# JoernZheng/parallel-data-compression-and-decompression

Hardware: AMD Instinct MI355X
Metric: compress+decompress GB/s (raw bytes / (deflate + inflate time)), .zwz bit-exact (higher is better)
Workload: dtype u8; 1 GPU; 10000 x 262144 B text-like files per GPU -> 50000 chunks of <=65535 B (BASELINE configs[2]); chunk_bytes=65535, max_batch_chunks=51200, parallelism=shard-per-gpu x1

## Files before the change

### parallel-data-compression-and-decompression_amd/csrc/lz_band.h

```cpp
#pragma once
#include "lz_core.h"

namespace zwz {

constexpr uint32_t kBand = kMaxChain;
constexpr uint32_t kBandNoLink = 0xffffu;
constexpr uint32_t kBandHaloWord = 0xffff0000u;

constexpr uint32_t kDenseSample = 2048;
ZWZ_HD bool sample_is_dense(uint32_t repeats, uint32_t thirds, uint32_t sampled, uint32_t L) {
    if (repeats == 0u || sampled == 0u) return false;
    if (thirds >= repeats) return true;
    const float walk = ((float)repeats + 3.0f * (float)thirds * (float)repeats / (float)(repeats - thirds)) * (float)L / ((float)sampled * (float)sampled);
    return walk >= 3.6f;
}

ZWZ_HD uint32_t band_word(uint32_t h, uint32_t p) { return h << 16 | p; }
ZWZ_HD uint32_t band_pos(uint32_t w) { return w & 0xffffu; }
ZWZ_HD uint32_t band_hash(uint32_t w) { return w >> 16; }

ZWZ_HD bool band_valid(uint32_t own, uint32_t c) {
    const uint32_t d = own - c;
    return (own ^ c) < 0x10000u && d < kMaxDist && d != band_pos(own);
}
ZWZ_HD bool band_first_at_max_dist(uint32_t own, uint32_t c) {
    const uint32_t p = band_pos(own), q = band_pos(c);
    return band_hash(c) == band_hash(own) && q != 0u && p - q == kMaxDist && !(p >= kSlidePos && q <= kWSize);
}

template <class Lv = LzDefaultLevel, class SFn>
ZWZ_HD uint32_t band_count(SFn S, uint32_t u) {
    const uint32_t own = S(u);
    uint32_t k = 0;
#if defined(__HIP_DEVICE_COMPILE__)
#pragma unroll
#endif
    for (uint32_t step = kBand; step >= 1u; step >>= 1) {
        const uint32_t t = k + step;
        if (t <= kBand && band_valid(own, S(u - t))) k = t;
    }
    if (k == 0u && band_first_at_max_dist(own, S(u - 1u))) k = 1u;
    return k < Lv::max_chain ? k : Lv::max_chain;
}

ZWZ_HD uint32_t band_ctz64(uint32_t lo, uint32_t hi) {
#if defined(__HIP_DEVICE_COMPILE__)
    uint32_t t0, t1;
    asm("v_ffbl_b32 %0, %1" : "=v"(t0) : "v"(lo));
    asm("v_ffbl_b32 %0, %1" : "=v"(t1) : "v"(hi));
    t1 |= 32u;
    return t0 < t1 ? t0 : t1;
#else
    if (lo) return (uint32_t)__builtin_ctz(lo);
    if (hi) return 32u + (uint32_t)__builtin_ctz(hi);
    return 0xffffffffu;
#endif
}
ZWZ_HD uint32_t band_key(uint32_t own_lo, uint32_t own_hi, uint32_t c_lo, uint32_t c_hi, uint32_t k) {
    const uint32_t t = band_ctz64(own_lo ^ c_lo, own_hi ^ c_hi);
    return ((t & 0x78u) << 5) | (129u - k);
}
ZWZ_HD uint32_t band_key_masked(uint32_t own_lo, uint32_t own_hi, uint32_t c_lo, uint32_t c_hi, uint32_t m_lo, uint32_t m_hi, uint32_t k) {
    const uint32_t t = band_ctz64((own_lo ^ c_lo) & m_lo, (own_hi ^ c_hi) & m_hi);
    return ((t & 0x78u) << 5) | (129u - k);
}
ZWZ_HD uint32_t band_tail_bytes(bool pure, uint32_t lookahead) {
    const uint32_t nb = pure ? lookahead - 3u : lookahead;
    return nb < 8u ? nb : 8u;
}
ZWZ_HD uint32_t band_tail_mask(uint32_t nbytes, uint32_t word ) {
    const uint32_t nb = nbytes > 4u * word ? nbytes - 4u * word : 0u;
    return nb >= 4u ? 0xffffffffu : (1u << (8u * nb)) - 1u;
}
constexpr uint32_t kBandKeyNonePure = 0u;
constexpr uint32_t kBandKeyNoneImpure = 0x2ffu;
ZWZ_HD uint32_t band_key_len(uint32_t key) { return key >> 8; }
ZWZ_HD uint32_t band_key_k(uint32_t key) { return 129u - (key & 0xffu); }

ZWZ_HD uint32_t band_record(uint32_t key, bool pure, uint32_t p, uint32_t cand_pos, uint32_t tail_len = 0) {
    const uint32_t len = band_key_len(key) == 15u ? tail_len : band_key_len(key) + (pure ? 3u : 0u), dist = p - cand_pos;
    if (len == kMinMatch && dist > kTooFar) return 0u;
    return entry_pack(len, dist);
}

template <class Lv = LzDefaultLevel, class SFn>
ZWZ_HD void band_generic(const uint8_t* data, SFn S, uint32_t u, uint32_t cnt, uint32_t L, uint32_t& e128, uint32_t& e32) {
    const uint32_t p = band_pos(S(u)), lookahead = L - p;
    const uint32_t max_len = lookahead < kMaxMatch ? lookahead : kMaxMatch, nice = lookahead < Lv::nice ? lookahead : Lv::nice;
    uint32_t best = kMinMatch - 1u, best_pos = 0, snap = 0xffffffffu;
    for (uint32_t k = 1; k <= cnt; k++) {
        const uint32_t c = band_pos(S(u - k));
        const uint32_t len = match_len_from(data, c, p, 0u, max_len);
        if (len > best) { best = len; best_pos = c; }
        if (k == Lv::snap_chain) snap = best >= kMinMatch ? entry_pack(best, p - best_pos) : 0u;
        if (best >= nice) break;
    }
    e128 = best >= kMinMatch ? entry_pack(best, p - best_pos) : 0u;
    e32 = snap != 0xffffffffu ? snap : e128;
    if (entry_len(e128) == kMinMatch && entry_dist(e128) > kTooFar) e128 = 0;
    if (entry_len(e32) == kMinMatch && entry_dist(e32) > kTooFar) e32 = 0;
}

template <class Lv = LzDefaultLevel, class SFn, class LinkFn, class EFn>
ZWZ_HD void band_deep(const uint8_t* data, SFn S, LinkFn link, EFn E, uint32_t first_own, uint32_t u, uint32_t cnt, uint32_t k1,
                      uint32_t deep, uint32_t L, uint64_t own , uint32_t& e128,
                      uint32_t& e32 ) {
    const uint32_t p = band_pos(S(u)), lookahead = L - p;
    const uint32_t max_len = lookahead < kMaxMatch ? lookahead : kMaxMatch, nice = lookahead < Lv::nice ? lookahead : Lv::nice;
    uint32_t best = 0, best_pos = 0, snap = 0xffffffffu;
    uint32_t j = u - k1;
    for (;;) {
        const uint32_t k = u - j;
        if (k > Lv::snap_chain && snap == 0xffffffffu) snap = best ? entry_pack(best, p - best_pos) : 0u;
        const uint32_t c = band_pos(S(j));
        const uint32_t len = match_len_from(data, c, p, deep, max_len);
        if (len > best) { best = len; best_pos = c; if (len >= nice) break; }
        if (j >= first_own) {
            const uint32_t j2 = link(j);
            if (j2 == kBandNoLink || u - j2 > cnt) break;
            j = j2;
        } else {
            uint32_t k2 = k + 1u;
            while (k2 <= cnt && E(u - k2) != own) k2++;
            if (k2 > cnt) break;
            j = u - k2;
        }
    }
    e128 = entry_pack(best, p - best_pos);
    if (k1 <= Lv::snap_chain) e32 = snap != 0xffffffffu ? snap : e128;
}

template <uint32_t H, class Lv = LzDefaultLevel, class SFn, class LinkFn, class EFn>
ZWZ_HD void band_deep_batched(const uint8_t* data, SFn S, LinkFn link, EFn E, uint32_t first_own, uint32_t u, uint32_t cnt, uint32_t k1,
                              uint32_t deep, uint32_t L, uint64_t own, uint32_t& e128, uint32_t& e32, uint32_t* visited = nullptr) {
    static_assert(H >= 1, "a batch holds a sharer");
    const uint32_t p = band_pos(S(u)), lookahead = L - p;
    const uint32_t max_len = lookahead < kMaxMatch ? lookahead : kMaxMatch, nice = lookahead < Lv::nice ? lookahead : Lv::nice;
    auto next = [&](uint32_t j) -> uint32_t {
        if (j >= first_own) {
            const uint32_t j2 = link(j);
            return j2 == kBandNoLink || u - j2 > cnt ? kBandNoLink : j2;
        }
        uint32_t k2 = u - j + 1u;
        while (k2 <= cnt && E(u - k2) != own) k2++;
        return k2 > cnt ? kBandNoLink : u - k2;
    };
    uint32_t best = 0, best_pos = 0, snap = 0xffffffffu, seen = 0;
    uint32_t j = u - k1;
    bool walking = true;
    while (walking) {
        uint32_t jv[H], len[H], nv = 1;
        jv[0] = j;
        for (uint32_t h = 1; h < H; h++) {
            const uint32_t j2 = next(jv[h - 1u]);
            if (j2 == kBandNoLink) break;
            jv[h] = j2; nv++;
        }
        for (uint32_t h = 0; h < nv; h++) len[h] = match_len_from(data, band_pos(S(jv[h])), p, deep, max_len);
        bool alive = true;
        for (uint32_t h = 0; h < nv; h++) {
            if (!alive) break;
            if (u - jv[h] > Lv::snap_chain && snap == 0xffffffffu) snap = best ? entry_pack(best, p - best_pos) : 0u;
            if (len[h] > best) { best = len[h]; best_pos = band_pos(S(jv[h])); }
            seen++;
            alive = best < nice;
        }
        j = alive && nv == H ? next(jv[H - 1u]) : kBandNoLink;
        walking = j != kBandNoLink;
    }
    if (visited) *visited = seen;
    e128 = entry_pack(best, p - best_pos);
    if (k1 <= Lv::snap_chain) e32 = snap != 0xffffffffu ? snap : e128;
}

}
```

### parallel-data-compression-and-decompression_amd/csrc/zwz_band.hip

```cpp
#include <hip/hip_runtime.h>

#include "lz_band.h"
#include "zwz_kernels.h"
#include "zwz_device.h"

#ifndef ZWZ_BAND_EXP
#define ZWZ_BAND_EXP 0
#endif

#if ZWZ_BAND_EXP & 16
#define ZWZ_STAMP(ph) do { if (tid == 0) { const uint64_t now_ = __builtin_amdgcn_s_memtime(); atomicAdd(&tickets[16 + (ph)], (uint32_t)((now_ - stamp_) >> 8)); stamp_ = now_; } } while (0)
#else
#define ZWZ_STAMP(ph) do { } while (0)
#endif

namespace zwz {

constexpr uint32_t kDenseThreads = 256;
__global__ __launch_bounds__(kDenseThreads) void lz_dense_list_kernel(const uint8_t* __restrict__ in, const uint64_t* __restrict__ in_off,
                                                                      const uint32_t* __restrict__ in_len, uint32_t n, uint32_t* __restrict__ link_stat,
                                                                      uint32_t force ) {
    __shared__ uint32_t s_set[kDenseThreads / 64][2048];
    const uint32_t wave = threadIdx.x >> 6, lane = lane_id();
    uint32_t* set = s_set[wave];
    for (uint32_t c = blockIdx.x * (kDenseThreads / 64u) + wave; c < n; c += gridDim.x * (kDenseThreads / 64u)) {
        const uint32_t L = in_len[c];
        bool dense = force == 2u && L != 0u;
        if (!dense && L >= kMinMatch) {
            for (uint32_t i = lane; i < 2048u; i += 64u) set[i] = 0;
            __builtin_amdgcn_fence(__ATOMIC_ACQ_REL, "wavefront");
            const uint32_t* d32 = reinterpret_cast<const uint32_t*>(in + in_off[c]);
            const uint32_t sampled = min(L - (kMinMatch - 1u), kDenseSample), nd = ((L + 15u) & ~15u) >> 2;
            uint32_t repeats = 0, thirds = 0;
            static_assert(kDenseSample == 2048, "eight trips of 256 positions, their loads asked for together");
            uint32_t w0[8], w1[8];
#pragma unroll
            for (uint32_t t = 0; t < 8; t++) {
                const uint32_t i = 64u * t + lane;
                w0[t] = 256u * t < sampled && i < nd ? d32[i] : 0u; w1[t] = 256u * t < sampled && i + 1u < nd ? d32[i + 1u] : 0u;
            }
#pragma unroll
            for (uint32_t t = 0; t < 8; t++) {
                if (256u * t >= sampled) break;
#pragma unroll
                for (uint32_t j = 0; j < 4; j++) {
                    const uint32_t x = j ? __builtin_amdgcn_alignbyte(w1[t], w0[t], j) : w0[t];
                    const uint32_t h = hash3(x & 0xffu, (x >> 8) & 0xffu, (x >> 16) & 0xffu);
                    const bool live = 256u * t + 4u * lane + j < sampled;
                    uint32_t old = 0, old2 = 0;
                    if (live) old = atomicOr(&set[h >> 5], 1u << (h & 31u));
                    const bool again = live && ((old >> (h & 31u)) & 1u);
                    if (again) old2 = atomicOr(&set[1024u + (h >> 5)], 1u << (h & 31u));
                    repeats += (uint32_t)__popcll(__builtin_amdgcn_ballot_w64(again));
                    thirds += (uint32_t)__popcll(__builtin_amdgcn_ballot_w64(again && ((old2 >> (h & 31u)) & 1u)));
                }
            }
            dense = sample_is_dense(repeats, thirds, sampled, L);
            __builtin_amdgcn_fence(__ATOMIC_ACQ_REL, "wavefront");
        }
        if (lane == 0) link_stat[c] = dense ? kDenseMark : 0u;
    }
}

__global__ __launch_bounds__(1024) void lz_lists_kernel(const uint32_t* __restrict__ in_len, const uint32_t* __restrict__ link_stat, uint32_t n,
                                                        uint32_t* __restrict__ dense_list, uint32_t* __restrict__ sparse_list, uint32_t* __restrict__ tickets) {
    __shared__ uint32_t s_d[16], s_s[16];
    const uint32_t tid = threadIdx.x, lane = lane_id(), wave = tid >> 6;
    uint32_t nd = 0, ns = 0;
    for (uint32_t c0 = 0; c0 < n; c0 += 1024u) {
        const uint32_t c = c0 + tid;
        const bool live = c < n && in_len[c] != 0u, dense = live && link_stat[c] == kDenseMark, sparse = live && !dense;
        const uint64_t md = __builtin_amdgcn_ballot_w64(dense), ms = __builtin_amdgcn_ballot_w64(sparse);
        if (lane == 0) { s_d[wave] = (uint32_t)__popcll(md); s_s[wave] = (uint32_t)__popcll(ms); }
        __syncthreads();
        uint32_t bd = nd, bs = ns, td = 0, ts = 0;
        for (uint32_t w = 0; w < 16u; w++) { bd += w < wave ? s_d[w] : 0u; bs += w < wave ? s_s[w] : 0u; td += s_d[w]; ts += s_s[w]; }
        if (dense) dense_list[bd + rank_in(md)] = c;
        if (sparse) sparse_list[bs + rank_in(ms)] = c;
        nd += td; ns += ts;
        __syncthreads();
    }
    if (tid == 0) { tickets[kTicketDenseCount] = nd; tickets[kTicketSparseCount] = ns; }
}

#ifndef ZWZ_SORT_DEPTH
#define ZWZ_SORT_DEPTH 16
#endif
constexpr uint32_t kSortDepth = ZWZ_SORT_DEPTH;
__global__ __launch_bounds__(kSortThreads) void lz_sort_kernel(const uint8_t* __restrict__ in, const uint64_t* __restrict__ in_off,
                                                               const uint32_t* __restrict__ in_len, const uint32_t* __restrict__ list,
                                                               uint32_t* __restrict__ tickets, uint32_t* __restrict__ sorted,
                                                               uint16_t* __restrict__ hbuf ,
                                                               uint32_t* __restrict__ scratch ) {
    __shared__ __attribute__((aligned(16))) uint32_t tab[16384];
    __shared__ uint32_t s_wsum[kSortThreads / 64];
    __shared__ uint32_t s_chunk;
    const uint32_t tid = threadIdx.x, lane = lane_id(), wave = __builtin_amdgcn_readfirstlane(tid >> 6);
    const uint32_t n_list = tickets[kTicketDenseCount];
    for (;;) {
        __syncthreads();
        if (tid == 0) s_chunk = atomicAdd(&tickets[kTicketSortNext], 1u);
        __syncthreads();
        const uint32_t t = s_chunk;
        if (t >= n_list) break;
        const uint32_t chunk = list[t];
        const uint32_t L = in_len[chunk];
        const uint32_t n = L >= kMinMatch ? L - (kMinMatch - 1u) : 0u;
        if (n == 0) continue;
        const uint32_t* d32 = reinterpret_cast<const uint32_t*>(in + in_off[chunk]);
        const uint32_t nd = ((L + 15u) & ~15u) >> 2;
        uint16_t* hb = hbuf + (size_t)chunk * kLinkStride;
        uint16_t* out = reinterpret_cast<uint16_t*>(sorted + (size_t)chunk * kSortedStride);
        {
            uint4* t4 = reinterpret_cast<uint4*>(tab);
            for (uint32_t i = tid; i < 4096u; i += kSortThreads) t4[i] = make_uint4(0, 0, 0, 0);
        }
        __syncthreads();
        {
            const uint4* d4 = reinterpret_cast<const uint4*>(d32);
            const uint32_t nv = nd >> 2;
#pragma unroll 1
            for (uint32_t i0 = tid; 16u * i0 < n; i0 += 8u * kSortThreads) {
                uint4 v[8]; uint32_t nx[8];
#pragma unroll
                for (uint32_t r = 0; r < 8; r++) {
                    const uint32_t i = i0 + r * kSortThreads;
                    v[r] = i < nv ? d4[i] : make_uint4(0, 0, 0, 0);
                    nx[r] = i + 1u < nv ? d32[4u * i + 4u] : 0u;
                }
#pragma unroll
                for (uint32_t r = 0; r < 8; r++) {
                    const uint32_t i = i0 + r * kSortThreads;
                    if (16u * i >= n) break;
                    const uint32_t w[5] = {v[r].x, v[r].y, v[r].z, v[r].w, nx[r]};
                    uint32_t h[16];
#pragma unroll
                    for (uint32_t j = 0; j < 16; j++) {
                        const uint32_t x = (j & 3u) ? __builtin_amdgcn_alignbyte(w[(j >> 2) + 1u], w[j >> 2], j & 3u) : w[j >> 2];
                        h[j] = hash3(x & 0xffu, (x >> 8) & 0xffu, (x >> 16) & 0xffu);
                        if (16u * i + j < n) atomicAdd(&tab[h[j] >> 1], (h[j] & 1u) ? 0x10000u : 1u);
                    }
#pragma unroll
                    for (uint32_t j = 0; j < 16; j++) h[j] = (h[j] >> 1) << 2 | (h[j] & 1u);
                    uint4* hb4 = reinterpret_cast<uint4*>(hb + 16u * i);
                    hb4[0] = make_uint4(h[0] | h[1] << 16, h[2] | h[3] << 16, h[4] | h[5] << 16, h[6] | h[7] << 16);
                    hb4[1] = make_uint4(h[8] | h[9] << 16, h[10] | h[11] << 16, h[12] | h[13] << 16, h[14] | h[15] << 16);
                }
            }
        }
        __syncthreads();
        {
            const uint32_t w_base = wave * 4096u;
            uint32_t tot = 0;
            for (uint32_t r = 0; r < 64u; r++) { const uint32_t v = tab[w_base + r * 64u + lane]; tot += (v & 0xffffu) + (v >> 16); }
            tot = wave_scan_incl(tot);
            if (lane == 63) s_wsum[wave] = tot;
            __syncthreads();
            uint32_t carry = 0;
            for (uint32_t i = 0; i < kSortThreads / 64u; i++) carry += i < wave ? s_wsum[i] : 0u;
            for (uint32_t r = 0; r < 64u; r++) {
                const uint32_t idx = w_base + r * 64u + lane;
                const uint32_t v = tab[idx], lo = v & 0xffffu, hi = v >> 16, own = lo + hi;
                const uint32_t incl = wave_scan_incl(own), ex = carry + incl - own;
                tab[idx] = ex | (ex + lo) << 16;
                carry += (uint32_t)__builtin_amdgcn_readlane((int)incl, 63);
            }
        }
        __syncthreads();
        if (wave == 0) {
            constexpr uint32_t K = kSortDepth;
            const uint32_t full = n / (64u * K);
            auto bump = [&](uint32_t w) { return atomicAdd(reinterpret_cast<uint32_t*>(reinterpret_cast<uint8_t*>(tab) + (w & 0xfffcu)), 1u << ((w & 1u) << 4)); };
            const uint16_t* hin = hb + lane;
            uint16_t* o = out + lane;
            uint32_t hv[K];
            auto ask = [&](uint32_t* h8) {
#pragma unroll
                for (uint32_t j = 0; j < K; j++) h8[j] = hin[j * 64u];
                hin += 64u * K;
            };
            if (full) ask(hv);
            uint32_t hp[K], op[K];
            for (uint32_t t = 0; t < full; t++) {
                uint32_t hn[K], old[K];
                if (t + 1u < full) ask(hn);
#pragma unroll
                for (uint32_t j = 0; j < K; j++) old[j] = bump(hv[j]);
                if (t) {
#pragma unroll
                    for (uint32_t j = 0; j < K; j++) o[j * 64u] = (uint16_t)(op[j] >> ((hp[j] & 1u) << 4));
                    o += 64u * K;
                }
#pragma unroll
                for (uint32_t j = 0; j < K; j++) { hp[j] = hv[j]; op[j] = old[j]; hv[j] = hn[j]; }
            }
            if (full) {
#pragma unroll
                for (uint32_t j = 0; j < K; j++) o[j * 64u] = (uint16_t)(op[j] >> ((hp[j] & 1u) << 4));
            }
            for (uint32_t p = full * 64u * K + lane; p - lane < n; p += 64u) {
                if (p < n) {
                    const uint32_t w = hb[p];
                    out[p] = (uint16_t)(bump(w) >> ((w & 1u) << 4));
                }
            }
        }
        if (scratch) {
            __syncthreads();
            uint4* o4 = reinterpret_cast<uint4*>(scratch + (size_t)chunk * kLazyScratchWords + kLazyBendOff);
            const uint4* t4 = reinterpret_cast<const uint4*>(tab);
            for (uint32_t i = tid; i < 4096u; i += kSortThreads) o4[i] = t4[i];
        }
    }
}

__global__ __launch_bounds__(kPlaceThreads) void lz_place_kernel(const uint32_t* __restrict__ in_len, const uint32_t* __restrict__ list,
                                                                 uint32_t* __restrict__ tickets, uint32_t* __restrict__ sorted) {
    extern __shared__ __attribute__((aligned(16))) uint8_t smem[];
    uint16_t* stage = reinterpret_cast<uint16_t*>(smem);
    __shared__ uint32_t s_chunk;
    const uint32_t tid = threadIdx.x;
    const uint32_t n_list = tickets[kTicketDenseCount];
    for (;;) {
        __syncthreads();
        if (tid == 0) s_chunk = atomicAdd(&tickets[kTicketPlaceNext], 1u);
        __syncthreads();
        const uint32_t t = s_chunk;
        if (t >= n_list) break;
        const uint32_t chunk = list[t];
        const uint32_t L = in_len[chunk];
        const uint32_t n = L >= kMinMatch ? L - (kMinMatch - 1u) : 0u;
        const uint4* d4 = reinterpret_cast<const uint4*>(sorted + (size_t)chunk * kSortedStride);
        uint4* o4 = reinterpret_cast<uint4*>(reinterpret_cast<uint16_t*>(sorted + (size_t)chunk * kSortedStride) + 65536);
        uint4 d[8];
#pragma unroll
        for (uint32_t r = 0; r < 8; r++) if (8u * (tid + kPlaceThreads * r) < n) d[r] = d4[tid + kPlaceThreads * r];
#pragma unroll
        for (uint32_t r = 0; r < 8; r++) {
            const uint32_t p0 = 8u * (tid + kPlaceThreads * r);
            const uint32_t dw[4] = {d[r].x, d[r].y, d[r].z, d[r].w};
#pragma unroll
            for (uint32_t j = 0; j < 8; j++) if (p0 + j < n) stage[(dw[j >> 1] >> (16u * (j & 1u))) & 0xffffu] = (uint16_t)(p0 + j);
        }
        __syncthreads();
        for (uint32_t i = tid; 8u * i < n; i += kPlaceThreads) o4[i] = reinterpret_cast<const uint4*>(stage)[i];
    }
}

constexpr uint32_t kBandArr = kBandTile + kBand;
constexpr uint32_t kBandDataBytes = 65536 + 64;
constexpr uint32_t kBandOffS = kBandDataBytes, kBandOffE = kBandOffS + kBandArr * 4, kBandOffCk = kBandOffE + kBandArr * 8,
                   kBandOffHas = kBandOffCk + kBandTile * 2;
static_assert(kBandOffHas + 8192 == kBandLdsBytes, "lz_match_band LDS layout");
static_assert(kBandTile % 64 == 0 && kBandOffE % 8 == 0 && kBandOffS % 16 == 0 && kBandOffCk % 16 == 0, "lz_match_band LDS alignment");
constexpr uint32_t kBandRuns = kBandTile / 8;

#ifndef ZWZ_BAND_WAVES
#define ZWZ_BAND_WAVES 4
#endif
#ifndef ZWZ_BAND_P2_BATCH
#define ZWZ_BAND_P2_BATCH 4
#endif
constexpr uint32_t kP2Batch = ZWZ_BAND_P2_BATCH;
static_assert(kP2Batch >= 1 && kP2Batch <= 32, "lz_match_band: sharers a batch");
template <class Lv>
__global__ __launch_bounds__(kBandThreads, ZWZ_BAND_WAVES) void lz_match_band_kernel(const uint8_t* __restrict__ in, const uint64_t* __restrict__ in_off,
                                                                    const uint32_t* __restrict__ in_len, const uint32_t* __restrict__ list,
                                                                    uint32_t* __restrict__ tickets, const uint32_t* __restrict__ sorted,
                                                                    uint2* __restrict__ entries, uint64_t* __restrict__ has128) {
    extern __shared__ __attribute__((aligned(16))) uint8_t smem[];
    uint8_t* sdata = smem;
    uint32_t* S = reinterpret_cast<uint32_t*>(smem + kBandOffS);
    uint2* E = reinterpret_cast<uint2*>(smem + kBandOffE);
    uint16_t* ck = reinterpret_cast<uint16_t*>(smem + kBandOffCk);
    uint32_t* hasb = reinterpret_cast<uint32_t*>(smem + kBandOffHas);
    uint16_t* flist = reinterpret_cast<uint16_t*>(E + kBand);
    __shared__ uint32_t s_chunk, s_grp[2], s_nflag, s_nrun;
    __shared__ uint16_t s_halo_link[kBand];
    __shared__ uint32_t s_bin[132];
    __shared__ uint16_t s_order[kBandRuns];
#if ZWZ_BAND_EXP & 16
    __shared__ uint64_t s_p2_start;
#endif
    const uint32_t tid = threadIdx.x, lane = lane_id(), wave = __builtin_amdgcn_readfirstlane(tid >> 6);
    const uint32_t n_list = tickets[kTicketDenseCount];
    for (uint32_t i = tid; i < 2048u; i += kBandThreads) hasb[i] = 0;
#if ZWZ_BAND_EXP & 16
    uint64_t stamp_ = __builtin_amdgcn_s_memtime();
#endif
    for (;;) {
        __syncthreads();
        ZWZ_STAMP(7);
        if (tid == 0) s_chunk = atomicAdd(&tickets[kTicketBandNext], 1u);
        __syncthreads();
        const uint32_t tk = s_chunk;
        if (tk >= n_list) break;
        const uint32_t chunk = list[tk];
        const uint32_t L = in_len[chunk];
        const uint32_t n = L >= kMinMatch ? L - (kMinMatch - 1u) : 0u;
        uint2* ent = entries + (size_t)chunk * kEntryStride;
        uint64_t* hm = has128 + (size_t)chunk * kMaskWords;
        const uint4* spos4 = reinterpret_cast<const uint4*>(reinterpret_cast<const uint16_t*>(sorted + (size_t)chunk * kSortedStride) + 65536);
        copy_vec16(reinterpret_cast<uint4*>(sdata), reinterpret_cast<const uint4*>(in + in_off[chunk]), (L + 15u) >> 4);
        ZWZ_STAMP(0);
        bool prev_pure = false;
        auto spos_of = [&](uint32_t a_) { return 8u * tid < kBandArr && 8u * tid + a_ >= kBand && 8u * tid + a_ - kBand < n ? spos4[(8u * tid + a_ - kBand) >> 3] : make_uint4(0, 0, 0, 0); };
        static_assert(kBandArr <= 8u * kBandThreads, "a thread holds eight of a tile's positions");
        uint4 v_next = spos_of(0u);
        for (uint32_t a = 0; a < n; a += kBandTile) {
            const uint32_t b = min(a + kBandTile, n), m = b - a + kBand;
            if (a < kBand) for (uint32_t i = tid; i < kBand - a; i += kBandThreads) S[i] = kBandHaloWord;
            if (tid == 0) { s_grp[0] = 0; s_grp[1] = 0; s_nflag = 0; s_nrun = 0; }
            if (tid < 132u) s_bin[tid] = 0;
            __syncthreads();
            bool mixed = false;
            {
                const uint32_t pw[4] = {v_next.x, v_next.y, v_next.z, v_next.w};
                if (8u * tid + a >= kBand) {
                    uint32_t prev_w = 0, prev_t = 0;
#pragma unroll
                    for (uint32_t j = 0; j < 8; j++) {
                        const uint32_t p = (pw[j >> 1] >> (16u * (j & 1u))) & 0xffffu;
                        const uint32_t* d = reinterpret_cast<const uint32_t*>(sdata) + (p >> 2);
                        const uint32_t w0 = d[0], w1 = d[1], w2 = d[2], w3 = d[3];
                        const uint32_t x = __builtin_amdgcn_alignbyte(w1, w0, p & 3u) & 0xffffffu;
                        const uint32_t word = band_word(hash3(x & 0xffu, (x >> 8) & 0xffu, x >> 16), p);
                        const bool up = (p & 3u) != 0u;
                        const uint32_t ea = up ? w1 : w0, eb = up ? w2 : w1, ec = up ? w3 : w2, sh = (p + 3u) & 3u;
                        if (8u * tid + j < m) {
                            S[8u * tid + j] = word;
                            E[8u * tid + j] = make_uint2(__builtin_amdgcn_alignbyte(eb, ea, sh), __builtin_amdgcn_alignbyte(ec, eb, sh));
                            if (j) mixed |= band_hash(word) == band_hash(prev_w) && x != prev_t;
                        }
                        prev_w = word; prev_t = x;
                    }
                }
                v_next = spos_of(a + kBandTile);
            }
            __syncthreads();
            ZWZ_STAMP(1);
            bool pure;
            {
                const uint32_t i = 8u * tid;
                if (i && i < m) {
                    const uint32_t w = S[i], wp = S[i - 1u];
                    const uint32_t tg = load_u32(sdata, band_pos(w)), tp = load_u32(sdata, band_pos(wp));
                    mixed |= w != kBandHaloWord && wp != kBandHaloWord && band_hash(w) == band_hash(wp) && ((tg ^ tp) & 0xffffffu) != 0u;
                }
                pure = !__syncthreads_or((int)mixed);
                if (!pure) {
                    for (uint32_t i2 = tid; i2 < m; i2 += kBandThreads) { const uint32_t q = band_pos(S[i2]); E[i2] = make_uint2(load_u32(sdata, q), load_u32(sdata, q + 4u)); }
                }
            }
            const uint32_t off = pure ? 3u : 0u, deep = pure ? 11u : 8u;
            auto Sf = [&](uint32_t i) { return S[i]; };
            ZWZ_STAMP(2);
            {
                constexpr uint32_t kOwnPer = (kBandTile + kBandThreads - 1) / kBandThreads;
                constexpr uint32_t kCap = Lv::max_chain;
                static_assert(kCap <= kBand && (kCap & (kCap - 1u)) == 0u, "the count is a binary search over [0, max_chain] inside the halo");
                uint32_t own[kOwnPer], k[kOwnPer];
#pragma unroll
                for (uint32_t j = 0; j < kOwnPer; j++) { const uint32_t i = kBand + tid + kBandThreads * j; own[j] = i < m ? S[i] : kBandHaloWord; k[j] = 0; }
                auto search_step = [&](uint32_t step) {
                    uint32_t c[kOwnPer];
#pragma unroll
                    for (uint32_t j = 0; j < kOwnPer; j++) { const uint32_t t = k[j] + step; c[j] = S[kBand + tid + kBandThreads * j - (t <= kCap ? t : 0u)]; }
#pragma unroll
                    for (uint32_t j = 0; j < kOwnPer; j++) { const uint32_t t = k[j] + step; if (t <= kCap && band_valid(own[j], c[j])) k[j] = t; }
                };
                search_step(kCap);
                bool open = false;
#pragma unroll
                for (uint32_t j = 0; j < kOwnPer; j++) open |= kBand + tid + kBandThreads * j < m && k[j] != kCap;
                if (__builtin_amdgcn_ballot_w64(open) != 0) {
#pragma unroll
                    for (uint32_t step = kCap / 2u; step >= 1u; step >>= 1) search_step(step);
                }
#pragma unroll
                for (uint32_t j = 0; j < kOwnPer; j++) {
                    const uint32_t i = kBand + tid + kBandThreads * j;
                    if (i < m) {
                        if (k[j] == 0u && band_first_at_max_dist(own[j], S[i - 1u])) k[j] = 1u;
                        ck[i - kBand] = (uint16_t)k[j];
                    }
                }
            }
            __syncthreads();
            ZWZ_STAMP(3);
            const bool halo_links = a == 0u || prev_pure == pure;
            if (tid < kBand) reinterpret_cast<uint16_t*>(S)[2u * tid + 1u] = a != 0u && halo_links ? s_halo_link[tid] : (uint16_t)kBandNoLink;
            prev_pure = pure;
            const uint32_t n_run = (b - a + 7u) >> 3;
            uint32_t run_key = 0;
            if (tid < n_run) {
                const uint4 c8 = *reinterpret_cast<const uint4*>(ck + 8u * tid);
                const uint32_t cw[4] = {c8.x, c8.y, c8.z, c8.w};
#pragma unroll
                for (uint32_t j = 0; j < 8; j++) if (8u * tid + j < b - a) run_key = max(run_key, (cw[j >> 1] >> (16u * (j & 1u))) & 0xffu);
                if (run_key) atomicAdd(&s_bin[128u - run_key], 1u);
            }
            __syncthreads();
            if (wave == 0) {
                const uint32_t v0 = s_bin[lane], v1 = s_bin[64u + lane];
                const uint32_t i0 = wave_scan_incl(v0), t0 = (uint32_t)__builtin_amdgcn_readlane((int)i0, 63);
                const uint32_t i1 = wave_scan_incl(v1);
                s_bin[lane] = i0 - v0; s_bin[64u + lane] = t0 + i1 - v1;
                if (lane == 63) s_nrun = t0 + i1;
            }
            __syncthreads();
            if (tid < n_run && run_key) s_order[atomicAdd(&s_bin[128u - run_key], 1u)] = (uint16_t)tid;
            __syncthreads();
            ZWZ_STAMP(8);
            const uint32_t n_act = s_nrun, n_grp = (n_act + 7u) >> 3;
            const uint32_t none = pure ? kBandKeyNonePure : kBandKeyNoneImpure;
            for (;;) {
                uint32_t g = 0;
                if (lane == 0) g = atomicAdd(&s_grp[0], 1u);
                g = __builtin_amdgcn_readfirstlane(g);
                if (g >= n_grp) break;
                const uint32_t ri = 8u * g + (lane >> 3);
                const uint32_t i = kBand + 8u * (ri < n_act ? (uint32_t)s_order[ri] : 0u) + (lane & 7u);
                const bool active = ri < n_act && i < m;
                const uint32_t w = S[i], p = band_pos(w);
                const uint32_t cntb = active ? (uint32_t)ck[i - kBand] : 0u;
                const uint2 own = E[i];
                const uint32_t kmax = (ZWZ_BAND_EXP & 2) ? 0u : (uint32_t)__builtin_amdgcn_readlane((int)wave_scan_max_incl(cntb), 63);
                const uint32_t kmin = 128u - (uint32_t)__builtin_amdgcn_readlane((int)wave_scan_max_incl(cntb ? 128u - cntb : 0u), 63);
                uint32_t best = cntb ? none : 0xffffffffu, snap = none;
                const uint2* Ei = E + i;
                auto key_of = [&](const uint2 c, uint32_t kc) {
                    uint32_t t0, t1, a1, key;
                    asm("v_ffbl_b32 %0, %1" : "=v"(t0) : "v"(own.x ^ c.x));
                    asm("v_ffbl_b32 %0, %1" : "=v"(t1) : "v"(own.y ^ c.y));
                    asm("v_and_or_b32 %0, %1, %2, 32" : "=v"(a1) : "v"(t1), "s"(0x78u));
                    const uint32_t m8 = min(t0 & 0x78u, a1);
                    asm("v_lshl_or_b32 %0, %1, 5, %2" : "=v"(key) : "v"(m8), "s"(kc));
                    return key;
                };
                const uint32_t la = L - p;
                const bool tail = active && la < deep;
                if (__builtin_amdgcn_ballot_w64(tail) == 0) {
                    uint32_t k0 = 0;
                    for (; k0 + 8u <= kmin; k0 += 8u) {
                        uint2 c[8];
#pragma unroll
                        for (uint32_t j = 0; j < 8; j++) c[j] = Ei[-(int)(k0 + j + 1u)];
#pragma unroll
                        for (uint32_t j = 0; j < 8; j += 2) {
                            const uint32_t ka = key_of(c[j], 128u - k0 - j), kb = key_of(c[j + 1], 127u - k0 - j);
                            asm("v_max3_u32 %0, %0, %1, %2" : "+v"(best) : "v"(ka), "v"(kb));
                        }
                        if (k0 + 8u == Lv::snap_chain) snap = best;
                    }
                    for (; k0 < kmax; k0 += 8u) {
                        uint2 c[8];
#pragma unroll
                        for (uint32_t j = 0; j < 8; j++) c[j] = Ei[-(int)(k0 + j + 1u)];
#pragma unroll
                        for (uint32_t j = 0; j < 8; j++) {
                            const uint32_t key = key_of(c[j], 128u - k0 - j);
                            best = max(best, k0 + j + 1u <= cntb ? key : 0u);
                        }
                        if (k0 + 8u == Lv::snap_chain) snap = best;
                    }
                } else {
                    const uint32_t nb = tail ? band_tail_bytes(pure, la) : 8u, m_lo = band_tail_mask(nb, 0), m_hi = band_tail_mask(nb, 1);
                    for (uint32_t k = 1; k <= kmax; k++) {
                        const uint2 c = Ei[-(int)k];
                        const uint32_t key = band_key_masked(own.x, own.y, c.x, c.y, m_lo, m_hi, k);
                        best = max(best, k <= cntb ? key : 0u);
                        if (k == Lv::snap_chain) snap = best;
                    }
                }
                if (cntb == 0u) best = none;
                const uint32_t key32 = cntb > Lv::snap_chain ? snap : best;
                uint32_t e128 = 0, e32 = 0, k1 = 0;
                if (best != none) {
                    if (band_key_len(best) == 15u && !tail && !(ZWZ_BAND_EXP & 1)) k1 = band_key_k(best);
                    else e128 = band_record(best, pure, p, band_pos(S[i - band_key_k(best)]), la);
                }
                if (key32 != none && (tail || band_key_len(key32) != 15u)) e32 = band_record(key32, pure, p, band_pos(S[i - band_key_k(key32)]), la);
                if (active) {
                    if (k1) {
                        ck[i - kBand] = (uint16_t)(cntb | k1 << 8);
                        reinterpret_cast<uint16_t*>(S)[2u * i + 1u] = (uint16_t)(i - k1);
                        if (k1 > Lv::snap_chain && !(ZWZ_BAND_EXP & 4)) reinterpret_cast<uint32_t*>(ent + p)[1] = e32;
                        atomicOr(&hasb[p >> 5], 1u << (p & 31u));
                    } else {
                        reinterpret_cast<uint16_t*>(S)[2u * i + 1u] = (uint16_t)kBandNoLink;
                        if (e128) {
                            if (!(ZWZ_BAND_EXP & 4)) ent[p] = make_uint2(e128, e32); else asm volatile("" :: "v"(e128), "v"(e32), "v"(p));
                            atomicOr(&hasb[p >> 5], 1u << (p & 31u));
                        }
                    }
                }
            }
            for (uint32_t i = kBand + tid; i < m; i += kBandThreads) if ((uint32_t)ck[i - kBand] == 0u) reinterpret_cast<uint16_t*>(S)[2u * i + 1u] = (uint16_t)kBandNoLink;
            __syncthreads();
            ZWZ_STAMP(4);
            for (uint32_t i = kBand + tid; i - tid < m; i += kBandThreads) {
                const bool f = i < m && ((uint32_t)ck[i - kBand] >> 8) != 0u;
                const uint64_t fm = __builtin_amdgcn_ballot_w64(f);
                if (fm) {
                    uint32_t base = 0;
                    if (lane == 0) base = atomicAdd(&s_nflag, (uint32_t)__popcll(fm));
                    base = __builtin_amdgcn_readfirstlane(base);
                    if (f) flist[base + rank_in(fm)] = (uint16_t)i;
                }
            }
#if ZWZ_BAND_EXP & 16
            if (tid == 0) s_p2_start = __builtin_amdgcn_s_memtime();
#endif
            __syncthreads();
            ZWZ_STAMP(9);
            const uint32_t n_flag = s_nflag;
            for (;;) {
                uint32_t g = 0;
                if (lane == 0) g = atomicAdd(&s_grp[1], 1u);
                g = __builtin_amdgcn_readfirstlane(g);
                if (64u * g >= n_flag) break;
#if ZWZ_BAND_EXP & 16
                if (lane == 0 && g == ((n_flag + 63u) >> 6) / 2u) atomicAdd(&tickets[16 + 10], (uint32_t)((__builtin_amdgcn_s_memtime() - s_p2_start) >> 8));
#endif
                const bool on = 64u * g + lane < n_flag;
                const uint32_t i = on ? (uint32_t)flist[64u * g + lane] : kBand;
                const uint32_t c = ck[i - kBand], cnt = c & 0xffu, k1 = c >> 8;
                const uint32_t p = band_pos(S[i]), la = L - p;
                const uint32_t max_len = la < kMaxMatch ? la : kMaxMatch, nice = la < Lv::nice ? la : Lv::nice;
                const uint32_t own2_lo = load_u32(sdata, p + deep), own2_hi = load_u32(sdata, p + deep + 4u);
                const uint32_t own3_lo = load_u32(sdata, p + deep + 8u), own3_hi = load_u32(sdata, p + deep + 12u);
                uint32_t best = 0, best_pos = 0, snap = 0xffffffffu;
                uint32_t j = on ? i - k1 : kBand;
                uint32_t w = S[j];
                bool walking = on, slow = false;
                while (__builtin_amdgcn_ballot_w64(walking) != 0) {
                    uint32_t wv[kP2Batch], nv = walking ? 1u : 0u;
                    wv[0] = w;
                    bool more = walking;
#pragma unroll
                    for (uint32_t h = 1; h < kP2Batch; h++) {
                        const uint32_t link = wv[h - 1u] >> 16;
                        more = more && i - link <= cnt;
                        wv[h] = S[more ? link : kBand];
                        nv += more ? 1u : 0u;
                    }
                    const uint32_t link_n = wv[kP2Batch - 1u] >> 16;
                    const bool more_n = more && i - link_n <= cnt;
                    const uint32_t wn = S[more_n ? link_n : kBand];
                    bool alive = walking;
                    uint32_t jh = j;
#pragma unroll
                    for (uint32_t h = 0; h < kP2Batch; h++) {
                        const uint32_t q = band_pos(wv[h]), sh = (q + deep) & 3u;
                        const uint32_t* d = reinterpret_cast<const uint32_t*>(sdata) + ((q + deep) >> 2);
                        const uint32_t d0 = d[0], d1 = d[1], d2 = d[2], d3 = d[3], d4 = d[4];
                        uint32_t t0, t1, t2, t3;
                        asm("v_ffbl_b32 %0, %1" : "=v"(t0) : "v"(__builtin_amdgcn_alignbyte(d1, d0, sh) ^ own2_lo));
                        asm("v_ffbl_b32 %0, %1" : "=v"(t1) : "v"(__builtin_amdgcn_alignbyte(d2, d1, sh) ^ own2_hi));
                        asm("v_ffbl_b32 %0, %1" : "=v"(t2) : "v"(__builtin_amdgcn_alignbyte(d3, d2, sh) ^ own3_lo));
                        asm("v_ffbl_b32 %0, %1" : "=v"(t3) : "v"(__builtin_amdgcn_alignbyte(d4, d3, sh) ^ own3_hi));
                        const uint32_t tm = min(min(t0, t1 | 32u), min(t2 | 64u, t3 | 96u));
                        bool v = alive && h < nv;
                        if (!halo_links) { slow = slow || (v && jh < kBand); v = v && jh >= kBand; }
                        uint32_t l = deep + (tm >> 3);
                        if (v && tm == 0xffffffffu) l = match_len_from(sdata, q, p, deep + 16u, max_len);
                        l = l < max_len ? l : max_len;
                        if (v && i - jh > Lv::snap_chain && snap == 0xffffffffu) snap = best ? entry_pack(best, p - best_pos) : 0u;
                        if (v && l > best) { best = l; best_pos = q; }
                        alive = v && best < nice;
                        jh = wv[h] >> 16;
                    }
                    walking = alive && more_n;
                    j = link_n; w = wn;
                }
                uint32_t e128 = entry_pack(best, p - best_pos), e32 = snap != 0xffffffffu ? snap : e128;
                if (slow) {
                    const uint64_t own = (uint64_t)load_u32(sdata, p + off) | (uint64_t)load_u32(sdata, p + off + 4u) << 32;
                    band_deep<Lv>(sdata, Sf, [&](uint32_t jj) { return S[jj] >> 16; },
                              [&](uint32_t jj) { const uint2 e = E[jj]; return (uint64_t)e.x | (uint64_t)e.y << 32; },
                              kBand, i, cnt, k1, deep, L, own, e128, e32);
                }
                if (on) {
                    if (ZWZ_BAND_EXP & 4) asm volatile("" :: "v"(e128), "v"(e32), "v"(p));
                    if (!(ZWZ_BAND_EXP & 4)) {
                        reinterpret_cast<uint32_t*>(ent + p)[0] = e128;
                        if (k1 <= Lv::snap_chain) reinterpret_cast<uint32_t*>(ent + p)[1] = e32;
                    }
                }
            }
            __syncthreads();
            if (tid < kBand && b < n) {
                const uint32_t lk = S[m - kBand + tid] >> 16;
                s_halo_link[tid] = (uint16_t)(lk != kBandNoLink && lk >= m - kBand ? lk - (m - kBand) : kBandNoLink);
            }
            __syncthreads();
            ZWZ_STAMP(5);
        }
        __syncthreads();
        for (uint32_t i = tid; i < ((L + 63u) >> 6); i += kBandThreads) {
            hm[i] = (uint64_t)hasb[2 * i] | ((uint64_t)hasb[2 * i + 1] << 32);
            hasb[2 * i] = 0; hasb[2 * i + 1] = 0;
        }
        ZWZ_STAMP(6);
    }
}

uint32_t exp_flags_band() { return (uint32_t)(ZWZ_BAND_EXP); }

hipError_t configure_band_kernels() {
    hipError_t e = hipFuncSetAttribute(reinterpret_cast<const void*>(lz_place_kernel), hipFuncAttributeMaxDynamicSharedMemorySize, (int)kPlaceLdsBytes);
    if (e != hipSuccess) return e;
    e = hipFuncSetAttribute(reinterpret_cast<const void*>(lz_match_band_kernel<LzLevel<4>>), hipFuncAttributeMaxDynamicSharedMemorySize, (int)kBandLdsBytes);
    if (e != hipSuccess) return e;
    e = hipFuncSetAttribute(reinterpret_cast<const void*>(lz_match_band_kernel<LzLevel<5>>), hipFuncAttributeMaxDynamicSharedMemorySize, (int)kBandLdsBytes);
    if (e != hipSuccess) return e;
    return hipFuncSetAttribute(reinterpret_cast<const void*>(lz_match_band_kernel<LzLevel<6>>), hipFuncAttributeMaxDynamicSharedMemorySize, (int)kBandLdsBytes);
}

hipError_t launch_dense_list(const DeflateArgs& a, hipStream_t s, uint32_t which) {
    const uint32_t cus = a.cu_count ? a.cu_count : 256u, want = (a.n + kDenseThreads / 64u - 1u) / (kDenseThreads / 64u);
    hipLaunchKernelGGL(lz_dense_list_kernel, dim3(want < 8u * cus ? want : 8u * cus), dim3(kDenseThreads), 0, s, a.in, a.in_off, a.in_len, a.n, a.link_stat, which);
    hipLaunchKernelGGL(lz_lists_kernel, dim3(1), dim3(1024), 0, s, a.in_len, a.link_stat, a.n, a.dense_list, a.sparse_list, a.tickets);
    return hipGetLastError();
}

hipError_t launch_sort(const DeflateArgs& a, hipStream_t s) {
    const uint32_t cus = a.cu_count ? a.cu_count : 256u;
    const uint32_t G = a.n < 2u * cus ? a.n : 2u * cus;
    hipLaunchKernelGGL(lz_sort_kernel, dim3(G), dim3(kSortThreads), 0, s, a.in, a.in_off, a.in_len, a.dense_list, a.tickets, a.sorted, a.links,
                       reinterpret_cast<uint32_t*>(a.entries));
    return hipGetLastError();
}

hipError_t launch_place(const DeflateArgs& a, hipStream_t s) {
    const uint32_t cus = a.cu_count ? a.cu_count : 256u;
    const uint32_t G = a.n < cus ? a.n : cus;
    hipLaunchKernelGGL(lz_place_kernel, dim3(G), dim3(kPlaceThreads), kPlaceLdsBytes, s, a.in_len, a.dense_list, a.tickets, a.sorted);
    return hipGetLastError();
}

hipError_t launch_match_band(const DeflateArgs& a, hipStream_t s) {
    const uint32_t cus = a.cu_count ? a.cu_count : 256u;
    const uint32_t G = a.n < cus ? a.n : cus;
    switch (a.level) {
#define ZWZ_BAND_LAUNCH(N) case N: hipLaunchKernelGGL(lz_match_band_kernel<LzLevel<N>>, dim3(G), dim3(kBandThreads), kBandLdsBytes, s, a.in, a.in_off, a.in_len, a.dense_list, \
                                                 a.tickets, a.sorted, a.entries, a.has128); break;
        ZWZ_BAND_LAUNCH(4) ZWZ_BAND_LAUNCH(5) ZWZ_BAND_LAUNCH(6)
#undef ZWZ_BAND_LAUNCH
        default: return hipErrorInvalidValue;
    }
    return hipGetLastError();
}

}
```

Measured before the change: 22.22 GB/s.

## Pack two band-key candidates per VGPR with 16-bit SDWA ops and parameterise run size

New measurement: 23.36 GB/s, median of 6. 5.1% higher.

```diff
diff --git a/parallel-data-compression-and-decompression_amd/csrc/lz_band.h b/parallel-data-compression-and-decompression_amd/csrc/lz_band.h
--- a/parallel-data-compression-and-decompression_amd/csrc/lz_band.h
+++ b/parallel-data-compression-and-decompression_amd/csrc/lz_band.h
@@ -64,6 +64,40 @@
     const uint32_t t = band_ctz64((own_lo ^ c_lo) & m_lo, (own_hi ^ c_hi) & m_hi);
     return ((t & 0x78u) << 5) | (129u - k);
 }
+constexpr uint32_t kBandPairLenMask = 0x00780078u;
+ZWZ_HD uint32_t band_key_pair(uint32_t own_lo, uint32_t own_hi, uint32_t a_lo, uint32_t a_hi, uint32_t b_lo, uint32_t b_hi, uint32_t k, uint32_t mask) {
+    const uint32_t ta = band_ctz64(own_lo ^ a_lo, own_hi ^ a_hi) & 0xffffu, tb = band_ctz64(own_lo ^ b_lo, own_hi ^ b_hi) & 0xffffu;
+    return (((ta | tb << 16) & mask) << 5) | (129u - k) | (128u - k) << 16;
+}
+ZWZ_HD uint64_t band_trip_mask(uint32_t k0, uint32_t cnt) {
+    const int32_t over = (int32_t)(k0 + 8u) - (int32_t)cnt;
+    const uint32_t d = over < 0 ? 0u : over > 8 ? 8u : (uint32_t)over;
+    return 0x7878787878787878ull >> (8u * d < 63u ? 8u * d : 63u);
+}
+ZWZ_HD uint32_t band_pair_mask(uint64_t trip_mask, uint32_t j) {
+    return ((uint32_t)(trip_mask >> (8u * j)) & 0xffu) | ((uint32_t)(trip_mask >> (8u * j + 8u)) & 0xffu) << 16;
+}
+ZWZ_HD uint32_t band_pair_max(uint32_t pair) { return (pair & 0xffffu) > (pair >> 16) ? pair & 0xffffu : pair >> 16; }
+template <class Lv = LzDefaultLevel, class EFn>
+ZWZ_HD void band_first_pass(uint64_t own, EFn E, uint32_t cnt, uint32_t kmin, uint32_t kmax, uint32_t none, uint32_t& best, uint32_t& snap) {
+    const uint32_t own_lo = (uint32_t)own, own_hi = (uint32_t)(own >> 32);
+    uint32_t best2 = cnt ? none | none << 16 : 0xffffffffu;
+    snap = none;
+    for (uint32_t k0 = 0; k0 < kmax; k0 += 8u) {
+        const bool masked = k0 + 8u > kmin;
+        const uint64_t have = band_trip_mask(k0, cnt);
+        for (uint32_t j = 0; j < 8u; j += 2u) {
+            const uint64_t a = E(k0 + j + 1u), b = E(k0 + j + 2u);
+            const uint32_t key = band_key_pair(own_lo, own_hi, (uint32_t)a, (uint32_t)(a >> 32), (uint32_t)b, (uint32_t)(b >> 32), k0 + j + 1u,
+                                               masked ? band_pair_mask(have, j) : kBandPairLenMask);
+            const uint32_t lo = (key & 0xffffu) > (best2 & 0xffffu) ? key & 0xffffu : best2 & 0xffffu, hi = (key >> 16) > (best2 >> 16) ? key >> 16 : best2 >> 16;
+            best2 = lo | hi << 16;
+        }
+        if (k0 + 8u == Lv::snap_chain) snap = band_pair_max(best2);
+    }
+    best = cnt ? band_pair_max(best2) : none;
+}
+
 ZWZ_HD uint32_t band_tail_bytes(bool pure, uint32_t lookahead) {
     const uint32_t nb = pure ? lookahead - 3u : lookahead;
     return nb < 8u ? nb : 8u;
diff --git a/parallel-data-compression-and-decompression_amd/csrc/zwz_band.hip b/parallel-data-compression-and-decompression_amd/csrc/zwz_band.hip
--- a/parallel-data-compression-and-decompression_amd/csrc/zwz_band.hip
+++ b/parallel-data-compression-and-decompression_amd/csrc/zwz_band.hip
@@ -253,7 +253,13 @@
                    kBandOffHas = kBandOffCk + kBandTile * 2;
 static_assert(kBandOffHas + 8192 == kBandLdsBytes, "lz_match_band LDS layout");
 static_assert(kBandTile % 64 == 0 && kBandOffE % 8 == 0 && kBandOffS % 16 == 0 && kBandOffCk % 16 == 0, "lz_match_band LDS alignment");
-constexpr uint32_t kBandRuns = kBandTile / 8;
+#ifndef ZWZ_BAND_RUN
+#define ZWZ_BAND_RUN 8
+#endif
+constexpr uint32_t kBandRun = ZWZ_BAND_RUN;
+static_assert(kBandRun == 8 || kBandRun == 4 || kBandRun == 2, "lz_match_band: a run is 8, 4 or 2 entries");
+constexpr uint32_t kBandRuns = kBandTile / kBandRun, kBandRunsPer = (kBandRuns + kBandThreads - 1) / kBandThreads;
+static_assert(kBandLdsBytes + 1072u + 2u * kBandRuns <= 160u * 1024u, "lz_match_band: s_order does not fit beside the tile");
 
 #ifndef ZWZ_BAND_WAVES
 #define ZWZ_BAND_WAVES 4
@@ -391,14 +397,21 @@
             const bool halo_links = a == 0u || prev_pure == pure;
             if (tid < kBand) reinterpret_cast<uint16_t*>(S)[2u * tid + 1u] = a != 0u && halo_links ? s_halo_link[tid] : (uint16_t)kBandNoLink;
             prev_pure = pure;
-            const uint32_t n_run = (b - a + 7u) >> 3;
-            uint32_t run_key = 0;
-            if (tid < n_run) {
-                const uint4 c8 = *reinterpret_cast<const uint4*>(ck + 8u * tid);
-                const uint32_t cw[4] = {c8.x, c8.y, c8.z, c8.w};
-#pragma unroll
-                for (uint32_t j = 0; j < 8; j++) if (8u * tid + j < b - a) run_key = max(run_key, (cw[j >> 1] >> (16u * (j & 1u))) & 0xffu);
-                if (run_key) atomicAdd(&s_bin[128u - run_key], 1u);
+            const uint32_t n_run = (b - a + kBandRun - 1u) / kBandRun;
+            uint32_t run_key[kBandRunsPer];
+#pragma unroll
+            for (uint32_t t = 0; t < kBandRunsPer; t++) {
+                const uint32_t r = tid + kBandThreads * t;
+                run_key[t] = 0;
+                if (r < n_run) {
+                    uint32_t cw[4] = {0, 0, 0, 0};
+                    if constexpr (kBandRun == 8) { const uint4 c8 = *reinterpret_cast<const uint4*>(ck + 8u * r); cw[0] = c8.x; cw[1] = c8.y; cw[2] = c8.z; cw[3] = c8.w; }
+                    else if constexpr (kBandRun == 4) { const uint2 c4 = *reinterpret_cast<const uint2*>(ck + 4u * r); cw[0] = c4.x; cw[1] = c4.y; }
+                    else cw[0] = *reinterpret_cast<const uint32_t*>(ck + 2u * r);
+#pragma unroll
+                    for (uint32_t j = 0; j < kBandRun; j++) if (kBandRun * r + j < b - a) run_key[t] = max(run_key[t], (cw[j >> 1] >> (16u * (j & 1u))) & 0xffu);
+                    if (run_key[t]) atomicAdd(&s_bin[128u - run_key[t]], 1u);
+                }
             }
             __syncthreads();
             if (wave == 0) {
@@ -409,63 +422,75 @@
                 if (lane == 63) s_nrun = t0 + i1;
             }
             __syncthreads();
-            if (tid < n_run && run_key) s_order[atomicAdd(&s_bin[128u - run_key], 1u)] = (uint16_t)tid;
+#pragma unroll
+            for (uint32_t t = 0; t < kBandRunsPer; t++) if (run_key[t]) s_order[atomicAdd(&s_bin[128u - run_key[t]], 1u)] = (uint16_t)(tid + kBandThreads * t);
             __syncthreads();
             ZWZ_STAMP(8);
-            const uint32_t n_act = s_nrun, n_grp = (n_act + 7u) >> 3;
+            constexpr uint32_t kRunsWave = 64u / kBandRun;
+            const uint32_t n_act = s_nrun, n_grp = (n_act + kRunsWave - 1u) / kRunsWave;
             const uint32_t none = pure ? kBandKeyNonePure : kBandKeyNoneImpure;
             for (;;) {
                 uint32_t g = 0;
                 if (lane == 0) g = atomicAdd(&s_grp[0], 1u);
                 g = __builtin_amdgcn_readfirstlane(g);
                 if (g >= n_grp) break;
-                const uint32_t ri = 8u * g + (lane >> 3);
-                const uint32_t i = kBand + 8u * (ri < n_act ? (uint32_t)s_order[ri] : 0u) + (lane & 7u);
+                const uint32_t ri = kRunsWave * g + lane / kBandRun;
+                const uint32_t i = kBand + kBandRun * (ri < n_act ? (uint32_t)s_order[ri] : 0u) + (lane & (kBandRun - 1u));
                 const bool active = ri < n_act && i < m;
                 const uint32_t w = S[i], p = band_pos(w);
                 const uint32_t cntb = active ? (uint32_t)ck[i - kBand] : 0u;
                 const uint2 own = E[i];
                 const uint32_t kmax = (ZWZ_BAND_EXP & 2) ? 0u : (uint32_t)__builtin_amdgcn_readlane((int)wave_scan_max_incl(cntb), 63);
                 const uint32_t kmin = 128u - (uint32_t)__builtin_amdgcn_readlane((int)wave_scan_max_incl(cntb ? 128u - cntb : 0u), 63);
-                uint32_t best = cntb ? none : 0xffffffffu, snap = none;
+                uint32_t best, snap = none;
                 const uint2* Ei = E + i;
-                auto key_of = [&](const uint2 c, uint32_t kc) {
-                    uint32_t t0, t1, a1, key;
-                    asm("v_ffbl_b32 %0, %1" : "=v"(t0) : "v"(own.x ^ c.x));
-                    asm("v_ffbl_b32 %0, %1" : "=v"(t1) : "v"(own.y ^ c.y));
-                    asm("v_and_or_b32 %0, %1, %2, 32" : "=v"(a1) : "v"(t1), "s"(0x78u));
-                    const uint32_t m8 = min(t0 & 0x78u, a1);
-                    asm("v_lshl_or_b32 %0, %1, 5, %2" : "=v"(key) : "v"(m8), "s"(kc));
+                auto key2_of = [&](const uint2 ca, const uint2 cb, uint32_t tags, uint32_t mask) {
+                    uint32_t t0, t1, m, key;
+                    asm("v_ffbl_b32_sdwa %0, %1 dst_sel:WORD_0 dst_unused:UNUSED_PAD src0_sel:DWORD" : "=v"(t0) : "v"(own.x ^ ca.x));
+                    asm("v_ffbl_b32_sdwa %0, %1 dst_sel:WORD_1 dst_unused:UNUSED_PRESERVE src0_sel:DWORD" : "+v"(t0) : "v"(own.x ^ cb.x));
+                    asm("v_ffbl_b32_sdwa %0, %1 dst_sel:WORD_0 dst_unused:UNUSED_PAD src0_sel:DWORD" : "=v"(t1) : "v"(own.y ^ ca.y));
+                    asm("v_ffbl_b32_sdwa %0, %1 dst_sel:WORD_1 dst_unused:UNUSED_PRESERVE src0_sel:DWORD" : "+v"(t1) : "v"(own.y ^ cb.y));
+                    asm("v_pk_min_u16 %0, %1, %2" : "=v"(m) : "v"(t0), "v"(t1 | 0x00200020u));
+                    asm("v_lshl_or_b32 %0, %1, 5, %2" : "=v"(key) : "v"(m & mask), "s"(tags));
                     return key;
                 };
                 const uint32_t la = L - p;
                 const bool tail = active && la < deep;
                 if (__builtin_amdgcn_ballot_w64(tail) == 0) {
+                    uint32_t best2 = cntb ? none | none << 16 : 0xffffffffu, snap2 = none | none << 16;
+                    auto both = [](uint32_t x) { return max(x & 0xffffu, x >> 16); };
                     uint32_t k0 = 0;
                     for (; k0 + 8u <= kmin; k0 += 8u) {
                         uint2 c[8];
 #pragma unroll
                         for (uint32_t j = 0; j < 8; j++) c[j] = Ei[-(int)(k0 + j + 1u)];
+                        const uint32_t tg = (128u - k0) * 0x10001u;
 #pragma unroll
                         for (uint32_t j = 0; j < 8; j += 2) {
-                            const uint32_t ka = key_of(c[j], 128u - k0 - j), kb = key_of(c[j + 1], 127u - k0 - j);
-                            asm("v_max3_u32 %0, %0, %1, %2" : "+v"(best) : "v"(ka), "v"(kb));
+                            const uint32_t key = key2_of(c[j], c[j + 1], tg - (j * 0x10001u + 0x10000u), kBandPairLenMask);
+                            asm("v_pk_max_u16 %0, %0, %1" : "+v"(best2) : "v"(key));
                         }
-                        if (k0 + 8u == Lv::snap_chain) snap = best;
+                        if (k0 + 8u == Lv::snap_chain) snap2 = best2;
                     }
                     for (; k0 < kmax; k0 += 8u) {
                         uint2 c[8];
 #pragma unroll
                         for (uint32_t j = 0; j < 8; j++) c[j] = Ei[-(int)(k0 + j + 1u)];
-#pragma unroll
-                        for (uint32_t j = 0; j < 8; j++) {
-                            const uint32_t key = key_of(c[j], 128u - k0 - j);
-                            best = max(best, k0 + j + 1u <= cntb ? key : 0u);
+                        const uint32_t tg = (128u - k0) * 0x10001u;
+                        const uint64_t have = band_trip_mask(k0, cntb);
+#pragma unroll
+                        for (uint32_t j = 0; j < 8; j += 2) {
+                            const uint32_t hw = (uint32_t)(have >> (j & 4u ? 32 : 0));
+                            const uint32_t mask = __builtin_amdgcn_perm(hw, hw, j & 2u ? 0x0c030c02u : 0x0c010c00u);
+                            const uint32_t key = key2_of(c[j], c[j + 1], tg - (j * 0x10001u + 0x10000u), mask);
+                            asm("v_pk_max_u16 %0, %0, %1" : "+v"(best2) : "v"(key));
                         }
-                        if (k0 + 8u == Lv::snap_chain) snap = best;
-                    }
+                        if (k0 + 8u == Lv::snap_chain) snap2 = best2;
+                    }
+                    best = both(best2); snap = both(snap2);
                 } else {
                     const uint32_t nb = tail ? band_tail_bytes(pure, la) : 8u, m_lo = band_tail_mask(nb, 0), m_hi = band_tail_mask(nb, 1);
+                    best = none;
                     for (uint32_t k = 1; k <= kmax; k++) {
                         const uint2 c = Ei[-(int)k];
                         const uint32_t key = band_key_masked(own.x, own.y, c.x, c.y, m_lo, m_hi, k);
```
